# caki35/UNet-Torch

Hardware: AMD Instinct MI355X
Metric: images/sec training step, 4-level U-Net 1ch→2cls 512×512, at 1/2/4/8 MI355X (higher is better)
Workload: dtype f16

## Files before the change

unet-torch_amd/csrc/elementwise_f16.hip:

```cpp
#include "common.h"

typedef _Float16 half8 __attribute__((ext_vector_type(8)));

namespace {

static int rpb_for(long M) {
    long r = (M + 2047) / 2048;
    r = (r + 63) / 64 * 64;
    return (int)(r < 64 ? 64 : (r > 2048 ? 2048 : r));
}

inline bool al16(const void* p) { return (((uintptr_t)p) & 15) == 0; }

__global__ __launch_bounds__(256) void bn_bwd_reduce1_v8(const half_t* __restrict__ da, int ldda,
                                                         const half_t* __restrict__ y, int ldy,
                                                         const float4* __restrict__ tx, const float* __restrict__ rstd,
                                                         float* __restrict__ ws, long M, int C, int RPB) {
    __shared__ float red[2][256][9];
    const int tid = threadIdx.x;
    const int G = C >> 3;
    const int PL = 256 / G;
    const int cg = tid % G, pl = tid / G;
    const long r0 = (long)blockIdx.x * RPB;
    long r1 = r0 + RPB;
    if (r1 > M) r1 = M;
    float4 t[8];
    float rs[8];
#pragma unroll
    for (int j = 0; j < 8; ++j) { t[j] = tx[cg * 8 + j]; rs[j] = rstd[cg * 8 + j]; }
    float s[8], q[8];
#pragma unroll
    for (int j = 0; j < 8; ++j) s[j] = q[j] = 0.f;
#define UMI_BNB_ACC(yv_, gv_)                                          \
    _Pragma("unroll") for (int j = 0; j < 8; ++j) {                    \
        float yy = (float)yv_[j];                                      \
        float z = umi_tx_pre(yy, t[j]);                                \
        float dz = z > t[j].w ? (float)gv_[j] : 0.f;                   \
        s[j] += dz;                                                    \
        q[j] = fmaf(dz, (yy - t[j].x) * rs[j], q[j]);                  \
    }
    long r = r0 + pl;
    for (; r + PL < r1; r += 2 * PL) {
        half8 yv0 = *reinterpret_cast<const half8*>(y + r * ldy + cg * 8);
        half8 gv0 = *reinterpret_cast<const half8*>(da + r * ldda + cg * 8);
        half8 yv1 = *reinterpret_cast<const half8*>(y + (r + PL) * ldy + cg * 8);
        half8 gv1 = *reinterpret_cast<const half8*>(da + (r + PL) * ldda + cg * 8);
        UMI_BNB_ACC(yv0, gv0)
        UMI_BNB_ACC(yv1, gv1)
    }
    if (r < r1) {
        half8 yv = *reinterpret_cast<const half8*>(y + r * ldy + cg * 8);
        half8 gv = *reinterpret_cast<const half8*>(da + r * ldda + cg * 8);
        UMI_BNB_ACC(yv, gv)
    }
#undef UMI_BNB_ACC
#pragma unroll
    for (int j = 0; j < 8; ++j) { red[0][tid][j] = s[j]; red[1][tid][j] = q[j]; }
    __syncthreads();
    for (int i = tid; i < 2 * C; i += 256) {
        int which = i / C, c = i - which * C;
        int g = c >> 3, j = c & 7;
        float a = 0.f;
        for (int k = 0; k < PL; ++k) a += red[which][k * G + g][j];
        ws[((long)blockIdx.x * 2 + which) * C + c] = a;
    }
}

template <bool SQ = false>
__device__ __forceinline__ void colsum_v8_body(const half_t* __restrict__ x, int ldx, float* __restrict__ ws, long M, int C,
                                               int RPB) {
    __shared__ float red[256][9];
    float q0[8] = {0.f, 0.f, 0.f, 0.f, 0.f, 0.f, 0.f, 0.f};
    const int tid = threadIdx.x;
    const int Gt = C >> 3, gb = blockIdx.y * 256;
    const int Gb = Gt - gb < 256 ? Gt - gb : 256;
    const int PL = 256 / Gb;
    const int cgl = tid % Gb, pl = tid / Gb, cg = gb + cgl;
    const long r0 = (long)blockIdx.x * RPB;
    long r1 = r0 + RPB;
    if (r1 > M) r1 = M;
    float s0[8], s1[8];
#pragma unroll
    for (int j = 0; j < 8; ++j) s0[j] = s1[j] = 0.f;
    if (pl < PL) {
        long r = r0 + pl;
        for (; r + 3 * PL < r1; r += 4 * PL) {
            half8 a = *reinterpret_cast<const half8*>(x + r * ldx + cg * 8);
            half8 b = *reinterpret_cast<const half8*>(x + (r + PL) * ldx + cg * 8);
            half8 c = *reinterpret_cast<const half8*>(x + (r + 2 * PL) * ldx + cg * 8);
            half8 d = *reinterpret_cast<const half8*>(x + (r + 3 * PL) * ldx + cg * 8);
#pragma unroll
            for (int j = 0; j < 8; ++j) {
                s0[j] += (float)a[j] + (float)c[j]; s1[j] += (float)b[j] + (float)d[j];
                if (SQ) {
                    const float fa = (float)a[j], fb = (float)b[j], fc = (float)c[j], fd = (float)d[j];
                    q0[j] = fmaf(fa, fa, fmaf(fb, fb, fmaf(fc, fc, fmaf(fd, fd, q0[j]))));
                }
            }
        }
        for (; r < r1; r += PL) {
            half8 a = *reinterpret_cast<const half8*>(x + r * ldx + cg * 8);
#pragma unroll
            for (int j = 0; j < 8; ++j) { s0[j] += (float)a[j]; if (SQ) q0[j] = fmaf((float)a[j], (float)a[j], q0[j]); }
        }
    }
#pragma unroll
    for (int j = 0; j < 8; ++j) red[tid][j] = s0[j] + s1[j];
    __syncthreads();
    for (int cl = tid; cl < Gb * 8; cl += 256) {
        float a = 0.f;
        for (int k = 0; k < PL; ++k) a += red[k * Gb + (cl >> 3)][cl & 7];
        ws[((long)blockIdx.x * 2 + 0) * C + gb * 8 + cl] = a;
    }
    if (SQ) {
        __syncthreads();
#pragma unroll
        for (int j = 0; j < 8; ++j) red[tid][j] = q0[j];
        __syncthreads();
        for (int cl = tid; cl < Gb * 8; cl += 256) {
            float a = 0.f;
            for (int k = 0; k < PL; ++k) a += red[k * Gb + (cl >> 3)][cl & 7];
            ws[((long)blockIdx.x * 2 + 1) * C + gb * 8 + cl] = a;
        }
    }
}

template <bool SQ = false>
__global__ __launch_bounds__(256) void colsum_v8(const half_t* __restrict__ x, int ldx, float* __restrict__ ws, long M, int C,
                                                 int RPB) {
    colsum_v8_body<SQ>(x, ldx, ws, M, C, RPB);
}
struct CsGroup { const half_t* x[16]; float* out[16]; };
__global__ __launch_bounds__(256) void colsum_group_v8(CsGroup grp, int ldx, float* __restrict__ ws, long ws_stride, long M, int C,
                                                       int RPB) {
    colsum_v8_body<false>(grp.x[blockIdx.z], ldx, ws + blockIdx.z * ws_stride, M, C, RPB);
}
__global__ __launch_bounds__(256) void colsum_group_reduce(CsGroup grp, const float* __restrict__ ws, long ws_stride, int rows, int C,
                                                           float scale) {
    __shared__ double sh[4][64];
    const int cl = threadIdx.x & 63, rl = threadIdx.x >> 6;
    const int c = blockIdx.x * 64 + cl;
    const float* w = ws + blockIdx.y * ws_stride;
    double a = 0.0;
    if (c < C)
        for (int r = rl; r < rows; r += 4) a += (double)w[((long)r * 2 + 0) * C + c];
    sh[rl][cl] = a;
    __syncthreads();
    if (rl == 0 && c < C) grp.out[blockIdx.y][c] = (float)((sh[0][cl] + sh[1][cl] + sh[2][cl] + sh[3][cl]) * (double)scale);
}

__global__ __launch_bounds__(256) void bn_bwd_apply_v8(half_t* __restrict__ da, int ldda, const half_t* __restrict__ y,
                                                       int ldy, const float4* __restrict__ tx,
                                                       const float* __restrict__ rstd,
                                                       const float* __restrict__ sum_dz,
                                                       const float* __restrict__ sum_dzx, long M, int C) {
    const int G = C >> 3;
    const long gt = (long)blockIdx.x * 256 + threadIdx.x;
    const int cg = (int)(gt % G);
    const long stride_rows = ((long)gridDim.x * 256) / G;
    const float invM = 1.f / (float)M;
    float4 t[8];
    float rs[8], c1[8], c2[8];
#pragma unroll
    for (int j = 0; j < 8; ++j) {
        int c = cg * 8 + j;
        t[j] = tx[c];
        rs[j] = rstd[c];
        c1[j] = sum_dz[c] * invM;
        c2[j] = sum_dzx[c] * invM;
    }
    for (long r = gt / G; r < M; r += stride_rows) {
        half8 yv = *reinterpret_cast<const half8*>(y + r * ldy + cg * 8);
        half8 gv = *reinterpret_cast<const half8*>(da + r * ldda + cg * 8);
        *reinterpret_cast<half8*>(da + r * ldda + cg * 8) = umi_bn_dz8(yv, gv, t, rs, c1, c2);
    }
}

template <bool HAS_TX>
__global__ __launch_bounds__(256) void pool2_fwd_v8(const half_t* __restrict__ x, int ldx, const float4* __restrict__ tx,
                                                    half_t* __restrict__ y, int ldy, int N, int H, int W, int C) {
    const int G = C >> 3, Ho = H >> 1, Wo = W >> 1;
    const long gt = (long)blockIdx.x * 256 + threadIdx.x;
    const int cg = (int)(gt % G);
    const long stride_p = ((long)gridDim.x * 256) / G;
    const long P = (long)N * Ho * Wo;
    float4 t[8];
    if (HAS_TX) {
#pragma unroll
        for (int j = 0; j < 8; ++j) t[j] = tx[cg * 8 + j];
    }
    for (long p = gt / G; p < P; p += stride_p) {
        int wo = (int)(p % Wo);
        long r = p / Wo;
        int ho = (int)(r % Ho);
        int n = (int)(r / Ho);
        const half_t* base = x + ((long)((long)n * H + 2 * ho) * W + 2 * wo) * ldx + cg * 8;
        half8 v[4];
        v[0] = *reinterpret_cast<const half8*>(base);
        v[1] = *reinterpret_cast<const half8*>(base + ldx);
        v[2] = *reinterpret_cast<const half8*>(base + (long)W * ldx);
        v[3] = *reinterpret_cast<const half8*>(base + (long)W * ldx + ldx);
        half8 o;
#pragma unroll
        for (int j = 0; j < 8; ++j) {
            float m = -INFINITY;
#pragma unroll
            for (int d = 0; d < 4; ++d) {
                float f = (float)v[d][j];
                if (HAS_TX) f = umi_tx(f, t[j]);
                m = f > m ? f : m;
            }
            o[j] = (half_t)m;
        }
        *reinterpret_cast<half8*>(y + p * ldy + cg * 8) = o;
    }
}

template <bool HAS_TX, bool ACC, bool RED = false>
__global__ __launch_bounds__(256) void pool2_bwd_v8(const half_t* __restrict__ dp, int lddp, const half_t* __restrict__ x,
                                                    int ldx, const float4* __restrict__ tx, half_t* __restrict__ da,
                                                    int ldda, int N, int H, int W, int C,
                                                    const float* __restrict__ rstd = nullptr, float* __restrict__ ws = nullptr) {
    __shared__ float red[RED ? 2 : 1][RED ? 256 : 1][9];
    float rs[8], s[8], q[8];
#pragma unroll
    for (int j = 0; j < 8; ++j) rs[j] = s[j] = q[j] = 0.f;
    const int G = C >> 3, Ho = H >> 1, Wo = W >> 1;
    const long gt = (long)blockIdx.x * 256 + threadIdx.x;
    const int cg = (int)(gt % G);
    const long stride_p = ((long)gridDim.x * 256) / G;
    const long P = (long)N * Ho * Wo;
    float4 t[8];
    if (HAS_TX) {
#pragma unroll
        for (int j = 0; j < 8; ++j) t[j] = tx[cg * 8 + j];
    }
    if (RED) {
#pragma unroll
        for (int j = 0; j < 8; ++j) rs[j] = rstd[cg * 8 + j];
    }
    for (long p = gt / G; p < P; p += stride_p) {
        int wo = (int)(p % Wo);
        long r = p / Wo;
        int ho = (int)(r % Ho);
        int n = (int)(r / Ho);
        const long pix = ((long)((long)n * H + 2 * ho) * W + 2 * wo);
        const long off[4] = {0, 1, (long)W, (long)W + 1};
        half8 v[4];
#pragma unroll
        for (int d = 0; d < 4; ++d) v[d] = *reinterpret_cast<const half8*>(x + (pix + off[d]) * ldx + cg * 8);
        half8 g = *reinterpret_cast<const half8*>(dp + p * lddp + cg * 8);
        half8 o[4];
        if (ACC) {
#pragma unroll
            for (int d = 0; d < 4; ++d) o[d] = *reinterpret_cast<const half8*>(da + (pix + off[d]) * ldda + cg * 8);
        }
#pragma unroll
        for (int j = 0; j < 8; ++j) {
            float m = -INFINITY;
            int best = 0;
#pragma unroll
            for (int d = 0; d < 4; ++d) {
                float f = (float)v[d][j];
                if (HAS_TX) f = umi_tx(f, t[j]);
                if (d == 0 || f > m) { m = f; best = d; }
            }
#pragma unroll
            for (int d = 0; d < 4; ++d) {
                float add = (d == best) ? (float)g[j] : 0.f;
                o[d][j] = ACC ? (half_t)((float)o[d][j] + add) : (half_t)add;
                if (RED) {
                    const float yy = (float)v[d][j];
                    const float dz = umi_tx_pre(yy, t[j]) > t[j].w ? (float)o[d][j] : 0.f;
                    s[j] += dz;
                    q[j] = fmaf(dz, (yy - t[j].x) * rs[j], q[j]);
                }
            }
        }
#pragma unroll
        for (int d = 0; d < 4; ++d) *reinterpret_cast<half8*>(da + (pix + off[d]) * ldda + cg * 8) = o[d];
    }
    if (RED) {
        const int tid = threadIdx.x, PL = 256 / G;
#pragma unroll
        for (int j = 0; j < 8; ++j) { red[0][tid][j] = s[j]; red[1][tid][j] = q[j]; }
        __syncthreads();
        for (int i = tid; i < 2 * C; i += 256) {
            const int which = i / C, c = i - which * C;
            float a = 0.f;
            for (int k = 0; k < PL; ++k) a += red[which][k * G + (c >> 3)][c & 7];
            ws[((long)blockIdx.x * 2 + which) * C + c] = a;
        }
    }
}

bool vec_ok(int C, int lda, int ldb, const void* a, const void* b) {
    if (C % 8 || lda % 8 || ldb % 8) return false;
    const int G = C / 8;
    if (G > 256 || 256 % G) return false;
    return al16(a) && al16(b);
}

int grid_for(long items) {
    long g = (items + 255) / 256;
    if (g > 8192) g = 8192;
    if (g < 1) g = 1;
    return (int)g;
}

}

int umi_bn_bwd_rpb_f16v(long M) { return rpb_for(M); }

static int rpb_colsum(long M, int C) {
    const int G = C / 8 < 256 ? C / 8 : 256, PL = 256 / G;
    long r = (M + 1023) / 1024;
    if (r < 2 * PL) r = 2 * PL;
    r = (r + PL - 1) / PL * PL;
    return (int)(r > 4096 ? 4096 : r);
}
int umi_colsum_rows_f16v(long M, int C) { return (C % 8 == 0) ? (int)((M + rpb_colsum(M, C) - 1) / rpb_colsum(M, C)) : 0; }
bool umi_colsum_f16v(const void* x, int ldx, float* ws, long M, int C, hipStream_t s) {
    if (!umi_colsum_rows_f16v(M, C) || ldx % 8 || !al16(x)) return false;
    const int rpb = rpb_colsum(M, C);
    hipLaunchKernelGGL(colsum_v8<false>, dim3((unsigned)((M + rpb - 1) / rpb), (C / 8 + 255) / 256), dim3(256), 0, s, (const half_t*)x, ldx, ws,
                       M, C, rpb);
    return true;
}
bool umi_colsum_group_f16v(int n, const void* const* xs, int ldx, float* const* outs, float scale, float* ws, long M, int C,
                           hipStream_t s) {
    if (!umi_colsum_rows_f16v(M, C) || ldx % 8) return false;
    for (int i = 0; i < n; ++i)
        if (!al16(xs[i])) return false;
    int rpb = rpb_colsum(M, C);
    {
        const int cnt0 = n < 16 ? n : 16, G = C / 8 < 256 ? C / 8 : 256, PL = 256 / G;
        long r = (M * cnt0 * ((C / 8 + 255) / 256) + 1023) / 1024;
        r = (r + PL - 1) / PL * PL;
        if (r > rpb) rpb = (int)(r > 4096 ? 4096 : r);
    }
    const int rows = (int)((M + rpb - 1) / rpb);
    const long stride = (long)rows * 2 * C;
    for (int g0 = 0; g0 < n; g0 += 16) {
        const int cnt = n - g0 < 16 ? n - g0 : 16;
        CsGroup grp;
        for (int i = 0; i < 16; ++i) { const int j = g0 + (i < cnt ? i : 0); grp.x[i] = (const half_t*)xs[j]; grp.out[i] = outs[j]; }
        hipLaunchKernelGGL(colsum_group_v8, dim3((unsigned)rows, (C / 8 + 255) / 256, cnt), dim3(256), 0, s, grp, ldx, ws, stride, M, C, rpb);
        hipLaunchKernelGGL(colsum_group_reduce, dim3((C + 63) / 64, cnt), dim3(256), 0, s, grp, (const float*)ws, stride, rows, C, scale);
    }
    return true;
}
bool umi_bn_stats_f16v(const void* x, int ldx, float* part, long M, int C, hipStream_t s) {
    if (!umi_colsum_rows_f16v(M, C) || ldx % 8 || !al16(x)) return false;
    const int rpb = rpb_colsum(M, C);
    hipLaunchKernelGGL(colsum_v8<true>, dim3((unsigned)((M + rpb - 1) / rpb), (C / 8 + 255) / 256), dim3(256), 0, s, (const half_t*)x, ldx,
                       part, M, C, rpb);
    return true;
}

bool umi_bn_bwd_reduce1_f16v(const void* da, int ldda, const void* y, int ldy, const void* tx, const float* rstd, float* ws,
                             long M, int C, hipStream_t s) {
    if (!vec_ok(C, ldda, ldy, da, y)) return false;
    const int rpb = rpb_for(M);
    int rows = (int)((M + rpb - 1) / rpb);
    hipLaunchKernelGGL(bn_bwd_reduce1_v8, dim3(rows), dim3(256), 0, s, (const half_t*)da, ldda, (const half_t*)y, ldy,
                       (const float4*)tx, rstd, ws, M, C, rpb);
    return true;
}

bool umi_bn_bwd_apply_f16v(void* da, int ldda, const void* y, int ldy, const void* tx, const float* rstd,
                           const float* sum_dz, const float* sum_dzx, long M, int C, hipStream_t s) {
    if (!vec_ok(C, ldda, ldy, da, y)) return false;
    hipLaunchKernelGGL(bn_bwd_apply_v8, dim3(grid_for(M * (C / 8))), dim3(256), 0, s, (half_t*)da, ldda, (const half_t*)y, ldy,
                       (const float4*)tx, rstd, sum_dz, sum_dzx, M, C);
    return true;
}

bool umi_pool2_fwd_f16v(const void* x, int ldx, const void* tx, void* y, int ldy, int N, int H, int W, int C,
                        hipStream_t s) {
    if (!vec_ok(C, ldx, ldy, x, y)) return false;
    int grid = grid_for((long)N * (H / 2) * (W / 2) * (C / 8));
    if (tx) hipLaunchKernelGGL(pool2_fwd_v8<true>, dim3(grid), dim3(256), 0, s, (const half_t*)x, ldx, (const float4*)tx, (half_t*)y, ldy, N, H, W, C);
    else hipLaunchKernelGGL(pool2_fwd_v8<false>, dim3(grid), dim3(256), 0, s, (const half_t*)x, ldx, (const float4*)tx, (half_t*)y, ldy, N, H, W, C);
    return true;
}

int umi_pool2_bwd_bnred_rows(int N, int H, int W, int C) {
    if (((H | W) & 1) || C % 8 || C / 8 > 256 || 256 % (C / 8)) return 0;
    return grid_for((long)N * (H / 2) * (W / 2) * (C / 8));
}
bool umi_pool2_bwd_bnred_f16v(const void* dp, int lddp, const void* x, int ldx, const void* tx, const float* rstd, void* da,
                              int ldda, int accumulate, float* part, int N, int H, int W, int C, hipStream_t s) {
    if (!tx || !rstd || !part || !umi_pool2_bwd_bnred_rows(N, H, W, C)) return false;
    if (!vec_ok(C, ldx, ldda, x, da) || lddp % 8 || !al16(dp)) return false;
    const int grid = umi_pool2_bwd_bnred_rows(N, H, W, C);
    if (accumulate)
        hipLaunchKernelGGL((pool2_bwd_v8<true, true, true>), dim3(grid), dim3(256), 0, s, (const half_t*)dp, lddp, (const half_t*)x,
                           ldx, (const float4*)tx, (half_t*)da, ldda, N, H, W, C, rstd, part);
    else
        hipLaunchKernelGGL((pool2_bwd_v8<true, false, true>), dim3(grid), dim3(256), 0, s, (const half_t*)dp, lddp, (const half_t*)x,
                           ldx, (const float4*)tx, (half_t*)da, ldda, N, H, W, C, rstd, part);
    return true;
}

bool umi_pool2_bwd_f16v(const void* dp, int lddp, const void* x, int ldx, const void* tx, void* da, int ldda,
                        int accumulate, int N, int H, int W, int C, hipStream_t s) {
    if ((H | W) & 1) return false;
    if (!vec_ok(C, ldx, ldda, x, da) || lddp % 8 || !al16(dp)) return false;
    int grid = grid_for((long)N * (H / 2) * (W / 2) * (C / 8));
#define GO(T, A) hipLaunchKernelGGL((pool2_bwd_v8<T, A>), dim3(grid), dim3(256), 0, s, (const half_t*)dp, lddp, (const half_t*)x, ldx, (const float4*)tx, (half_t*)da, ldda, N, H, W, C, (const float*)nullptr, (float*)nullptr)
    if (tx) { if (accumulate) GO(true, true); else GO(true, false); }
    else    { if (accumulate) GO(false, true); else GO(false, false); }
#undef GO
    return true;
}
```

Baseline: 726.3.

## Restructure BN backward apply into row-blocked tiles with batched loads

The BN backward apply kernel now gives each workgroup a contiguous block of rows and a channel slice of up to 64 channel groups (a 2D grid). Per-channel constants are staged once in shared memory. Each lane issues several 16-byte loads before computing, with an asm barrier to keep the loads grouped. The goal is more memory-level parallelism, fewer 64-bit index computations and less redundant constant loading than the old grid-stride loop, at the cost of shared memory, extra registers and tuning macros.

```diff
diff --git a/unet-torch_amd/csrc/elementwise_f16.hip b/unet-torch_amd/csrc/elementwise_f16.hip
--- a/unet-torch_amd/csrc/elementwise_f16.hip
+++ b/unet-torch_amd/csrc/elementwise_f16.hip
@@ -149,30 +149,68 @@
     if (rl == 0 && c < C) grp.out[blockIdx.y][c] = (float)((sh[0][cl] + sh[1][cl] + sh[2][cl] + sh[3][cl]) * (double)scale);
 }
 
+#define BNA_GB 64
+#ifndef BNA_RT
+#define BNA_RT 4
+#endif
 __global__ __launch_bounds__(256) void bn_bwd_apply_v8(half_t* __restrict__ da, int ldda, const half_t* __restrict__ y,
                                                        int ldy, const float4* __restrict__ tx,
                                                        const float* __restrict__ rstd,
                                                        const float* __restrict__ sum_dz,
-                                                       const float* __restrict__ sum_dzx, long M, int C) {
+                                                       const float* __restrict__ sum_dzx, long M, int C, int RPW) {
+    __shared__ float4 s_t[8][BNA_GB];
+    __shared__ float s_k[3][8][BNA_GB];
+    const int tid = threadIdx.x;
     const int G = C >> 3;
-    const long gt = (long)blockIdx.x * 256 + threadIdx.x;
-    const int cg = (int)(gt % G);
-    const long stride_rows = ((long)gridDim.x * 256) / G;
+    const int Gb = G < BNA_GB ? G : BNA_GB;
+    const int PL = 256 / Gb;
+    const int cgl = tid & (Gb - 1), pl = tid / Gb;
+    const int cb = blockIdx.y * (Gb * 8);
     const float invM = 1.f / (float)M;
+    for (int i = tid; i < Gb * 8; i += 256) {
+        const int c = cb + i;
+        s_t[i & 7][i >> 3] = tx[c];
+        s_k[0][i & 7][i >> 3] = rstd[c];
+        s_k[1][i & 7][i >> 3] = sum_dz[c] * invM;
+        s_k[2][i & 7][i >> 3] = sum_dzx[c] * invM;
+    }
+    __syncthreads();
     float4 t[8];
     float rs[8], c1[8], c2[8];
 #pragma unroll
     for (int j = 0; j < 8; ++j) {
-        int c = cg * 8 + j;
-        t[j] = tx[c];
-        rs[j] = rstd[c];
-        c1[j] = sum_dz[c] * invM;
-        c2[j] = sum_dzx[c] * invM;
-    }
-    for (long r = gt / G; r < M; r += stride_rows) {
-        half8 yv = *reinterpret_cast<const half8*>(y + r * ldy + cg * 8);
-        half8 gv = *reinterpret_cast<const half8*>(da + r * ldda + cg * 8);
-        *reinterpret_cast<half8*>(da + r * ldda + cg * 8) = umi_bn_dz8(yv, gv, t, rs, c1, c2);
+        t[j] = s_t[j][cgl];
+        rs[j] = s_k[0][j][cgl];
+        c1[j] = s_k[1][j][cgl];
+        c2[j] = s_k[2][j][cgl];
+    }
+    const long r0 = (long)blockIdx.x * RPW;
+    long r1 = r0 + RPW;
+    if (r1 > M) r1 = M;
+    const int nr = (int)(r1 - r0);
+    half_t* dab = da + r0 * ldda + cb;
+    const half_t* yb = y + r0 * ldy + cb;
+    for (int r = pl; r < nr; r += BNA_RT * PL) {
+        unsigned oy[BNA_RT], og[BNA_RT];
+        half8 yv[BNA_RT], gv[BNA_RT];
+#pragma unroll
+        for (int k = 0; k < BNA_RT; ++k) {
+            const int q = r + k * PL < nr ? r + k * PL : nr - 1;
+            oy[k] = (unsigned)(q * ldy + cgl * 8);
+            og[k] = (unsigned)(q * ldda + cgl * 8);
+        }
+#pragma unroll
+        for (int k = 0; k < BNA_RT; ++k) {
+            yv[k] = *reinterpret_cast<const half8*>(yb + oy[k]);
+            gv[k] = *reinterpret_cast<const half8*>(dab + og[k]);
+        }
+#pragma unroll
+        for (int k = 0; k < BNA_RT; ++k) asm volatile("" : "+v"(yv[k]), "+v"(gv[k]));
+#pragma unroll
+        for (int k = 0; k < BNA_RT; ++k) {
+            const half8 o = umi_bn_dz8(yv[k], gv[k], t, rs, c1, c2);
+            if (r + k * PL < nr) *reinterpret_cast<half8*>(dab + og[k]) = o;
+        }
     }
 }
 
@@ -308,6 +346,22 @@
     return (int)g;
 }
 
+#ifndef BNA_WGS
+#define BNA_WGS 2048
+#endif
+#ifndef BNA_MIN_RL
+#define BNA_MIN_RL 8
+#endif
+#ifndef BNA_MAX_RL
+#define BNA_MAX_RL 64
+#endif
+int bna_rows_per_lane(long M, int PL, int gy) {
+    const long per_wg = (long)PL * (BNA_WGS / gy);
+    long rl = (M + per_wg - 1) / per_wg;
+    rl = (rl + BNA_RT - 1) / BNA_RT * BNA_RT;
+    return (int)(rl < BNA_MIN_RL ? BNA_MIN_RL : (rl > BNA_MAX_RL ? BNA_MAX_RL : rl));
+}
+
 }
 
 int umi_bn_bwd_rpb_f16v(long M) { return rpb_for(M); }
@@ -371,8 +425,11 @@
 bool umi_bn_bwd_apply_f16v(void* da, int ldda, const void* y, int ldy, const void* tx, const float* rstd,
                            const float* sum_dz, const float* sum_dzx, long M, int C, hipStream_t s) {
     if (!vec_ok(C, ldda, ldy, da, y)) return false;
-    hipLaunchKernelGGL(bn_bwd_apply_v8, dim3(grid_for(M * (C / 8))), dim3(256), 0, s, (half_t*)da, ldda, (const half_t*)y, ldy,
-                       (const float4*)tx, rstd, sum_dz, sum_dzx, M, C);
+    const int G = C / 8, Gb = G < BNA_GB ? G : BNA_GB, PL = 256 / Gb, gy = G / Gb;
+    const int rpw = bna_rows_per_lane(M, PL, gy) * PL;
+    if ((long)rpw * (ldda > ldy ? ldda : ldy) >= (1L << 30)) return false;
+    hipLaunchKernelGGL(bn_bwd_apply_v8, dim3((unsigned)((M + rpw - 1) / rpw), gy), dim3(256), 0, s, (half_t*)da, ldda,
+                       (const half_t*)y, ldy, (const float4*)tx, rstd, sum_dz, sum_dzx, M, C, rpw);
     return true;
 }
 
```

Result: faster. 741.3, median of 6 (+2.1%).
